# TuringLang/AdvancedVI.jl

Hardware: AMD Instinct MI355X
Metric: ELBO-grad-estimates/sec (higher is better)
Workload: dtype f32

## Files before the change

### advancedvi.jl_amd/csrc/kernels_fullrank_batch.hip

```cpp
#include <algorithm>
#include <cstdlib>
#include <type_traits>
#include <cstdio>
#include <vector>

#include "device_common.h"
#include "fr_elem.h"
#include "fr_planes.h"

#ifndef FB_VK
#define FB_VK 0
#endif
#ifndef FB_WJ
#define FB_WJ 1
#endif

namespace mivi {

struct FbArgs {
  int d, M, L;
  int dT, MT;
  const float *params;
  const float *t_mean, *t_istd;
  unsigned *CA;
  float *cscale;
  unsigned *epsP;
  unsigned *WV;
  float *winv;
  const float *t_prec;
  int dP;
  unsigned *PA;
  float *pscale;
  unsigned *RP;
  float *rinv;
  const float *Tinv;
  unsigned *TA;
  float *tscale;
  long long plane_stride;
  double *ell_part;
  long long ell_stride;
  double *he_part;
  long long he_stride;
  double *ld_part;
  const int4 *work;
  int n_work;
  float *grads;
  long long grad_stride;
  float *values;
  long long value_stride;
  float *grad_last, *value_last;
  int lane_last;
  int write_upper;
  int ent_kind, M_total;
  int *status;
  double ell_const;
  RngArgs rng;
  int n_riders;
  int obj;
  float *parts;
  long long part_stride;
  int knock;
  long long *dbg;
};
#ifdef MIVI_DEV
#define FB_STAMP(a, slot) do { if ((a).dbg && threadIdx.x == 0) (a).dbg[(size_t)blockIdx.x * 8 + (slot)] = (long long)wall_clock64(); } while (0)
#define FB_NOTE(a, slot, v) do { if ((a).dbg && threadIdx.x == 0) (a).dbg[(size_t)blockIdx.x * 8 + (slot)] = (long long)(v); } while (0)
#define FB_KNOCKED(a, b) ((a).knock & (b))
#else
#define FB_KNOCKED(a, b) false
#define FB_STAMP(a, slot) do { } while (0)
#define FB_NOTE(a, slot, v) do { } while (0)
#endif

template <int NT, class Ld4, class Ld>
__device__ __forceinline__ void fb_rowblock_planes(int d, int rb, int kg_lo, int kg_hi, int sub, int nsub, Ld4 ld4, Ld ld, unsigned *planes, float *scale, float *red) {
  constexpr int NP = NT / 8, NW = NT / 64;
  const int tid = threadIdx.x, r4 = tid & 7, part = tid >> 3, ng = d >> 4;
  f32x4 m = {0.f, 0.f, 0.f, 0.f};
  {
    int k = 16 * kg_lo + part;
    for (; k + 7 * NP <= 16 * kg_hi + 15; k += 8 * NP) {
      f32x4 v[8];
#pragma unroll
      for (int u = 0; u < 8; ++u) v[u] = ld4(k + NP * u, 32 * rb + 4 * r4);
#pragma unroll
      for (int u = 0; u < 8; ++u)
#pragma unroll
        for (int c = 0; c < 4; ++c) m[c] = fmaxf(m[c], fabsf(v[u][c]));
    }
    for (; k <= 16 * kg_hi + 15; k += NP) {
      const f32x4 v = ld4(k, 32 * rb + 4 * r4);
#pragma unroll
      for (int c = 0; c < 4; ++c) m[c] = fmaxf(m[c], fabsf(v[c]));
    }
  }
#pragma unroll
  for (int c = 0; c < 4; ++c) {
    m[c] = fmaxf(m[c], __shfl_xor(m[c], 8, 64));
    m[c] = fmaxf(m[c], __shfl_xor(m[c], 16, 64));
    m[c] = fmaxf(m[c], __shfl_xor(m[c], 32, 64));
  }
  if ((tid & 63) < 8) *(f32x4 *)(red + (tid >> 6) * 32 + 4 * r4) = m;
  lds_barrier();
  const int w = tid >> 6, lane = tid & 63, l31 = lane & 31, h = lane >> 5;
  float mm = red[l31];
#pragma unroll
  for (int p = 1; p < NW; ++p) mm = fmaxf(mm, red[p * 32 + l31]);
  float s, inv;
  fb_scale_of(mm, s, inv);
  if (sub == 0 && tid < 32) {
    scale[32 * rb + tid] = s;
    scale[d + 32 * rb + tid] = inv;
  }
  for (int kg = kg_lo + w + NW * sub; kg <= kg_hi; kg += NW * nsub) {
    float x[8];
#pragma unroll
    for (int e = 0; e < 8; ++e) x[e] = ld(16 * kg + 8 * (e >> 2) + 4 * h + (e & 3), 32 * rb + l31) * s;
    fb_store_frag(planes + ((size_t)rb * ng + kg) * kFrag + 4 * lane, x);
  }
}
template <int NT>
__device__ __forceinline__ void fb_cplanes_block(const FbArgs &a, int rb, int sub, int nsub, float *red) {
  const int d = a.d, ng = d >> 4, dT = a.dT;
  const float *C = a.params + dT;
  const int hi = 2 * rb + 3 < ng - 1 ? 2 * rb + 3 : ng - 1;
  if (dT == d) {
    fb_rowblock_planes<NT>(d, rb, 0, hi, sub, nsub,
                       [C, d](int k, int row) { f32x4 v = *(const f32x4 *)(C + (size_t)k * d + row);
#pragma unroll
                                                for (int c = 0; c < 4; ++c) v[c] = k > row + c ? 0.f : v[c];
                                                return v; },
                       [C, d](int k, int row) { const float v = C[(size_t)k * d + row]; return k > row ? 0.f : v; }, a.CA, a.cscale, red);
    return;
  }
  fb_rowblock_planes<NT>(d, rb, 0, hi, sub, nsub,
                     [C, dT](int k, int row) { const bool in = row < dT && k < dT;
                                               f32x4 v = *(const f32x4 *)(C + (size_t)(in ? k : 0) * dT + (in ? row : 0));
#pragma unroll
                                               for (int c = 0; c < 4; ++c) v[c] = (!in || k > row + c) ? 0.f : v[c];
                                               return v; },
                     [C, dT](int k, int row) { if (row >= dT || k > row) return 0.f; return C[(size_t)k * dT + row]; }, a.CA, a.cscale, red);
}
__global__ __launch_bounds__(512) void k_fb_pplanes(FbArgs a) {
  __shared__ float red[8 * 32];
  const float *P = a.t_prec;
  const int dP = a.dP;
  fb_rowblock_planes<512>(a.d, (int)blockIdx.x, 0, (a.d >> 4) - 1, (int)blockIdx.y, (int)gridDim.y,
                     [P, dP](int k, int row) { return *(const f32x4 *)(P + (size_t)k * dP + row); },
                     [P, dP](int k, int row) { return P[(size_t)k * dP + row]; }, a.PA, a.pscale, red);
}
__global__ __launch_bounds__(512) void k_fb_tplanes(FbArgs a) {
  __shared__ float red[8 * 32];
  const float *T = a.Tinv;
  const int d = a.d, rb = (int)blockIdx.x;
  fb_rowblock_planes<512>(d, rb, 2 * (rb & ~3), (d >> 4) - 1, (int)blockIdx.y, (int)gridDim.y,
                     [T, d](int k, int row) { f32x4 v = *(const f32x4 *)(T + (size_t)k * d + row);
#pragma unroll
                                              for (int c = 0; c < 4; ++c) v[c] = k >= row + c ? v[c] : 0.f;
                                              return v; },
                     [T, d](int k, int row) { const float v = T[(size_t)k * d + row]; return k >= row ? v : 0.f; }, a.TA, a.tscale, red);
}

__global__ __launch_bounds__(512) void k_fb_eps(FbArgs a) {
  __shared__ double red[128];
  const int tid = threadIdx.x, d = a.d;
  if ((int)blockIdx.y < a.n_riders) {
    const int r = (int)blockIdx.y * (int)gridDim.x + (int)blockIdx.x;
    if (r < 4 * (d >> 5)) fb_cplanes_block<512>(a, (d >> 5) - 1 - (r >> 2), r & 3, 4, (float *)red);
    return;
  }
  const int l = (int)blockIdx.y - a.n_riders, eb = 2 * (int)blockIdx.x + (tid >> 8);
  const uint64_t idx = rng_index(a.rng) + (a.obj ? 0ull : (uint64_t)l);
  const int moff = a.rng.m_offset + (a.obj ? l * a.MT : 0);
  unsigned *epsP = a.epsP + (size_t)l * a.plane_stride;
  const int nrb6 = d >> 6;
  const int R64 = eb % nrb6, c32 = eb / nrb6;
  const int lane = tid & 63, l31 = lane & 31, h = lane >> 5, f = (tid >> 6) & 3;
  const int rm = c32 * 32 + l31;
  const uint64_t q0 = (uint64_t)(moff + rm) * (uint64_t)(a.dT >> 2);
  float x[8], he = 0.f;
#pragma unroll
  for (int b = 0; b < 2; ++b) {
    const int ri = R64 * 64 + 4 * (4 * f + 2 * b + h);
    float e[4];
    eps_block<float>(a.rng.seed, idx, q0 + (uint64_t)(ri >> 2), e);
    if (!(ri < a.dT && rm < a.MT)) { e[0] = 0.f; e[1] = 0.f; e[2] = 0.f; e[3] = 0.f; }
#pragma unroll
    for (int r = 0; r < 4; ++r) x[4 * b + r] = e[r] * kEpsScale;
    he += 0.5f * (e[0] * e[0] + e[1] * e[1] + e[2] * e[2] + e[3] * e[3]);
  }
  fb_store_frag(epsP + ((size_t)c32 * (d >> 4) + 4 * R64 + f) * kFrag + 4 * lane, x);
  const float hw = wave_sum_f32(he);
  if (lane == 0) red[tid >> 6] = (double)hw;
  lds_barrier();
  if ((tid & 255) == 0) {
    const double *r4 = red + 4 * (tid >> 8);
    a.he_part[(size_t)l * a.he_stride + eb] = ((r4[0] + r4[1]) + r4[2]) + r4[3];
  }
}

constexpr int kImgW = 32 * 36;
template <int WJ>
__device__ __forceinline__ void fb_sched_interleave() {
  constexpr int NM = 6 * WJ, ND = 4 + 2 * WJ, NV = 2 * WJ;
  static_for<0, NM>([&](auto K) {
    constexpr int k = decltype(K)::value;
    constexpr int nrd = (k + 1) * ND / NM - k * ND / NM;
    __builtin_amdgcn_sched_group_barrier(0x008, 1, 0);
    if constexpr (nrd > 0) __builtin_amdgcn_sched_group_barrier(0x100, nrd, 0);
    if constexpr (k < NV) __builtin_amdgcn_sched_group_barrier(0x020, 1, 0);
  });
}
using FbI0 = std::integral_constant<int, 0>;
using FbI1 = std::integral_constant<int, 1>;
using FbI2 = std::integral_constant<int, 2>;
using FbI3 = std::integral_constant<int, 3>;
using FbT = std::true_type;
using FbN = std::false_type;

template <int MASK>
__device__ __forceinline__ float fb_lane_max(float v) {
#pragma unroll
  for (int o = 1; o < 64; o <<= 1)
    if (MASK & o) v = fmaxf(v, __shfl_xor(v, o, 64));
  return v;
}

enum { FB_DIAG = 0, FB_DENSE_R = 1, FB_DENSE_G = 2, FB_STL_U = 3 };
template <int WJ, int MODE, int NRP>
__global__ __launch_bounds__(512 / WJ, (MODE == 2 && NRP == 4 && WJ == 1) ? 4 : 2 / WJ) void k_fb_prod(FbArgs a) {
  constexpr bool kDG = MODE == FB_DENSE_G, kSU = MODE == FB_STL_U, kDR = MODE == FB_DENSE_R;
  constexpr int LDC = 36, NF = WJ, kPW = 2 * WJ;
  constexpr int NW = 8 / WJ, NWN = 4 / WJ;
  constexpr int kBody = (NRP * kStageW > 16 * kImgW) ? NRP * kStageW : 16 * kImgW;
  constexpr bool kTabInBody = kDG && NRP * kStageW + 2048 <= kBody;
  constexpr int kTab = kDG ? (kTabInBody ? 128 : 2048 + 128) : 0;
  __shared__ __attribute__((aligned(16))) unsigned lds[kBody + 4 * 128 + NW * 64 + kTab];
  float *vec = reinterpret_cast<float *>(lds + kBody);
  float *red = vec + 4 * 128;
  float *rsv = red + NW * 64;
  float *tab = kTabInBody ? reinterpret_cast<float *>(lds + NRP * kStageW) : rsv + 128;
  const int tid = threadIdx.x, lane = tid & 63, l31 = lane & 31, h = lane >> 5;
  const int w = __builtin_amdgcn_readfirstlane(tid >> 6);
  const int wm = w / NWN, wn = w % NWN;
  const __attribute__((address_space(4))) int *wp = (const __attribute__((address_space(4))) int *)a.work + 4 * blockIdx.x;
  const int ln = wp[0], rc = wp[1], flags = wp[2];
  const int rb = rc & 0xffff, cb = rc >> 16;
  const int d = a.d, ng = d >> 4;
  const int row0 = rb * 128, col0 = cb * 128;
  const int R0 = row0 >> 5;
  const int g0 = kSU ? 2 * R0 : 0;
  const int G = kDG ? ng : (kSU ? ng - g0 : 2 * (R0 + 4));
  const unsigned *sp[NF];
  int gmax[NF];
#pragma unroll
  for (int f = 0; f < NF; ++f) {
    const int fs = NF * w + f, fr = fs & 3;
    if (fs < 4) {
      sp[f] = (kDG ? a.PA : (kSU ? a.TA : a.CA)) + ((size_t)(R0 + fr) * ng + g0) * kFrag + 4 * lane;
      gmax[f] = (!kDG && !kSU && 2 * (R0 + fr) + 3 < G - 1) ? 2 * (R0 + fr) + 3 : G - 1;
    } else {
      sp[f] = (kDG ? a.RP : a.epsP) + (size_t)ln * a.plane_stride + ((size_t)((col0 >> 5) + fr) * ng + g0) * kFrag + 4 * lane;
      gmax[f] = G - 1;
    }
  }
  int gd = 0;
  constexpr int kMaxNB = 16;
  float tv[4] = {0.f, 0.f, 0.f, 0.f}, tri[kDG ? kMaxNB : 1], trs = 0.f;
  auto load_tables = [&]() {
    if (tid < 128) {
      if constexpr (!kDG && !kSU) {
        const bool in = row0 + tid < a.dT;
        tv[0] = in ? a.params[row0 + tid] : 0.f;
        tv[1] = in ? a.t_mean[row0 + tid] : 0.f;
        if (MODE == FB_DIAG) tv[2] = in ? a.t_istd[row0 + tid] : 0.f;
      }
      const float *sc = kDG ? a.pscale : (kSU ? a.tscale : a.cscale);
      tv[3] = sc[d + row0 + tid];
      if constexpr (kDG) {
        const float *ri = a.rinv + (size_t)ln * (size_t)(d >> 7) * a.M + col0 + tid;
        const int NB = d >> 7;
#pragma unroll
        for (int b = 0; b < kMaxNB; ++b) tri[b] = ri[(size_t)(b < NB ? b : NB - 1) * a.M];
        trs = ri[(size_t)rb * a.M];
      }
    }
    asm volatile("" ::: "memory");
  };
  auto stage_tables = [&]() {
    if (tid < 128) {
      if constexpr (!kDG && !kSU) {
        vec[tid] = tv[0];
        vec[128 + tid] = tv[1];
        if (MODE == FB_DIAG) vec[256 + tid] = tv[2];
      }
      vec[384 + tid] = tv[3] * ((kDG) ? 1.f : kEpsInv);
      if constexpr (kDG) {
        const int NB = d >> 7;
        float u = tri[0], grow = 1.f;
#pragma unroll
        for (int b = 1; b < kMaxNB; ++b) {
          if (b < NB) {
            float ratio = u / tri[b];
            if (!(ratio <= 1099511627776.f)) ratio = 1099511627776.f;
            if (ratio > 1.f && grow * ratio > 1.2089258e24f) ratio = fmaxf(1.2089258e24f / grow, 1.f);
            if (ratio > 1.f) grow *= ratio;
            tab[(b - 1) * 128 + tid] = ratio;
            u = u / ratio;
          }
        }
        tab[(NB - 1) * 128 + tid] = u;
        rsv[tid] = trs;
      }
    }
  };
  auto issue = [&](int slot) {
#pragma unroll
    for (int f = 0; f < NF; ++f) {
      unsigned *dst = lds + slot * kStageW + (NF * w + f) * 512;
      FB_GLDS16(sp[f], dst, 0);
      FB_GLDS16(sp[f], dst, 1024);
      sp[f] += gd < gmax[f] ? kFrag : 0;
    }
    ++gd;
  };
  f32x16 acc[2][WJ];
#pragma unroll
  for (int i = 0; i < 2; ++i)
#pragma unroll
    for (int j = 0; j < WJ; ++j)
#pragma unroll
      for (int r = 0; r < 16; ++r) acc[i][j][r] = 0.f;
  const int r32[2] = {R0 + 2 * wm, R0 + 2 * wm + 1};
  const int Gw = (kDG || kSU) ? G : 2 * r32[1] + 2;
  auto after_group = [&](auto S, int g) {
    if constexpr (kDG && (decltype(S)::value & 3) == 3) {
      if (((g + 1) & 7) == 0) {
#pragma unroll
        for (int j = 0; j < WJ; ++j) {
          const float f = tab[((g >> 3) << 7) + 32 * (WJ * wn + j) + l31];
#pragma unroll
          for (int i = 0; i < 2; ++i) {
#pragma unroll
            for (int r = 0; r < 16; ++r) acc[i][j][r] *= f;
          }
        }
        asm volatile("" ::: "memory");
      }
    }
  };
  auto compute = [&](auto S, int g, const FbFrags<WJ> &F) {
    if (!FB_KNOCKED(a, 2)) fb_group<WJ>(F, acc);
    fb_sched_interleave<WJ>();
    after_group(S, g);
  };
  const unsigned lds0 = (unsigned)(uintptr_t)lds + 16u * lane;
  const unsigned ab_lo = lds0 + (2 * wm) * 2 * 1024, bb_lo = lds0 + (8 + WJ * wn * 2) * 1024;
  const unsigned ab_hi = ab_lo + 4 * kStageW * 4, bb_hi = bb_lo + 4 * kStageW * 4;
  (void)ab_hi; (void)bb_hi;
  auto step = [&](auto S, auto VM, auto ISS, int g, const FbFrags<WJ> &Fc, FbFrags<WJ> &Fn) {
    constexpr int sl = decltype(S)::value;
    fb_wait_vm<kPW * decltype(VM)::value>();
    if (!FB_KNOCKED(a, 8)) fb_barrier();
#ifdef MIVI_SB
    __builtin_amdgcn_sched_barrier(0);
#endif
    auto group_and_read = [&]() {
#ifndef MIVI_DEV
      if constexpr (WJ == 1) {
        constexpr int nx = (sl + 1) % NRP, off = (nx & 3) * kStageW * 4;
        fb_group_read_asm<off>(acc[0][0], acc[1][0], Fc, Fn, nx < 4 ? ab_lo : ab_hi, nx < 4 ? bb_lo : bb_hi);
        if constexpr (kDG && (sl & 3) == 3) {
          if (((g + 1) & 7) == 0) asm volatile("s_nop 15\n\ts_nop 7" : "+v"(acc[0][0]), "+v"(acc[1][0])::"memory");
        }
        after_group(S, g);
      } else
#endif
      {
        if (!FB_KNOCKED(a, 4)) fb_read_frags<WJ>(lds, (sl + 1) % NRP, wm, wn, lane, Fn);
        compute(S, g, Fc);
      }
    };
    if constexpr (decltype(ISS)::value) {
      if (!FB_KNOCKED(a, 1)) issue(sl);
      group_and_read();
    } else if (g < Gw) {
      group_and_read();
    }
  };
  FB_STAMP(a, 0);
  FB_NOTE(a, 4, G);
  load_tables();
  static_for<0, NRP>([&](auto S) { issue(decltype(S)::value); });
  fb_wait_vm<kPW * NRP>();
  stage_tables();
  fb_wait_vm<kPW * (NRP - 1)>();
  fb_barrier();
  FB_STAMP(a, 1);
  {
    FbFrags<WJ> F0, F1;
    fb_read_frags<WJ>(lds, 0, wm, wn, lane, F0);
    int g = 0;
    for (; g + NRP < G; g += NRP) {
      static_for<0, NRP>([&](auto S) {
        constexpr int sv = decltype(S)::value;
        if constexpr (sv % 2 == 0) step(S, std::integral_constant<int, NRP - 2>{}, FbT{}, g + sv, F0, F1);
        else step(S, std::integral_constant<int, NRP - 2>{}, FbT{}, g + sv, F1, F0);
      });
    }
    static_for<0, NRP - 1>([&](auto S) {
      constexpr int sv = decltype(S)::value;
      if constexpr (sv % 2 == 0) step(S, std::integral_constant<int, NRP - 2 - sv>{}, FbN{}, g + sv, F0, F1);
      else step(S, std::integral_constant<int, NRP - 2 - sv>{}, FbN{}, g + sv, F1, F0);
    });
    __builtin_amdgcn_s_waitcnt(0xc07f);
    if (g + NRP - 1 < Gw) compute(std::integral_constant<int, NRP - 1>{}, g + NRP - 1, F1);
  }
  f32x16 (&tot)[2][WJ] = acc;
  fb_barrier();
  FB_STAMP(a, 2);
  float *img = reinterpret_cast<float *>(lds) + w * (2 * WJ * kImgW);
  unsigned *WVl = a.WV + (size_t)ln * a.plane_stride;
  unsigned *RPl = a.RP + (size_t)ln * a.plane_stride;
  double *ellp = a.ell_part + (size_t)ln * a.ell_stride;
  const int ncb = a.M >> 5, nmg = a.M >> 4;
  const int ei4 = 4 * (lane & 7);
  float amax[2][4];
  float cmax[WJ][4];
#pragma unroll
  for (int i = 0; i < 2; ++i)
#pragma unroll
    for (int c = 0; c < 4; ++c) amax[i][c] = 0.f;
#pragma unroll
  for (int j = 0; j < WJ; ++j)
#pragma unroll
    for (int p = 0; p < 4; ++p) cmax[j][p] = 0.f;
#pragma unroll
  for (int i = 0; i < 2; ++i) {
    const int lr = 64 * wm + 32 * i;
    f32x4 mu = {0.f, 0.f, 0.f, 0.f}, tm = mu, tis = mu;
    const f32x4 zf = *(const f32x4 *)(vec + 384 + lr + ei4);
    if constexpr (!kDG && !kSU) {
      mu = *(const f32x4 *)(vec + lr + ei4);
      tm = *(const f32x4 *)(vec + 128 + lr + ei4);
      if constexpr (MODE == FB_DIAG) tis = *(const f32x4 *)(vec + 256 + lr + ei4);
    }
#pragma unroll
    for (int j = 0; j < WJ; ++j) {
      float *I = img + (i * WJ + j) * kImgW;
      const int cb32 = (col0 >> 5) + WJ * wn + j;
      const bool pad = 32 * r32[i] >= a.dT || 32 * cb32 >= a.MT;
#pragma unroll
      for (int q = 0; q < 4; ++q) {
        const f32x4 v = {tot[i][j][4 * q], tot[i][j][4 * q + 1], tot[i][j][4 * q + 2], tot[i][j][4 * q + 3]};
        *(f32x4 *)(I + l31 * LDC + 8 * q + 4 * h) = v;
      }
      if constexpr (kSU) {
        const float uf = vec[384 + lr + l31];
        const float wo = a.winv[(size_t)ln * (size_t)(a.M >> 7) * d + (size_t)cb * d + row0 + lr + l31];
#pragma unroll
        for (int g2 = 0; g2 < 2; ++g2) {
          const unsigned *src = WVl + ((size_t)r32[i] * nmg + 2 * cb32 + g2) * kFrag + 4 * lane;
          const u32x4v wh = *(const u32x4v *)src, wl = *(const u32x4v *)(src + 256);
#pragma unroll
          for (int e = 0; e < 8; ++e) {
            float *p = I + (16 * g2 + 8 * (e >> 2) + 4 * h + (e & 3)) * LDC + l31;
            const float x = __builtin_fmaf(*p, uf, fb_unsplit2(wh, wl, e) * wo);
            *p = x;
            amax[i][0] = fmaxf(amax[i][0], fabsf(x));
          }
        }
        continue;
      }
      double s = 0.0;
#pragma unroll
      for (int p = 0; p < 4; ++p) {
        const int en = 8 * p + (lane >> 3);
        const f32x4 v = *(const f32x4 *)(I + en * LDC + ei4) * zf;
        float ell = 0.f;
        f32x4 wv;
        if constexpr (MODE == FB_DIAG) {
          const f32x4 z = mu + v;
#pragma unroll
          for (int c = 0; c < 4; ++c) wv[c] = diag_target_elem(z[c], tm[c], tis[c], ell);
        } else if constexpr (kDR) {
          const f32x4 z = mu + v;
          wv = z - tm;
        } else {
          const unsigned *fr = RPl + ((size_t)cb32 * ng + 2 * r32[i] + (ei4 >> 4)) * kFrag + 4 * (en + 32 * ((ei4 >> 2) & 1)) + 2 * ((ei4 >> 3) & 1);
          const uint2 qh = *(const uint2 *)fr, ql = *(const uint2 *)(fr + 256);
          const float rs = rsv[32 * (WJ * wn + j) + en];
          const unsigned uh[2] = {qh.x, qh.y}, ul[2] = {ql.x, ql.y};
#pragma unroll
          for (int c = 0; c < 4; ++c) wv[c] = dense_target_elem(v[c], fb_unsplit2_word(uh[c >> 1], ul[c >> 1], c & 1) * rs, ell);
        }
        if (pad) { wv = f32x4{0.f, 0.f, 0.f, 0.f}; ell = 0.f; }
        *(f32x4 *)(I + en * LDC + ei4) = wv;
        if constexpr (kDR) {
          cmax[j][p] = fmaxf(cmax[j][p], fmaxf(fmaxf(fabsf(wv[0]), fabsf(wv[1])), fmaxf(fabsf(wv[2]), fabsf(wv[3]))));
        } else {
#pragma unroll
          for (int c = 0; c < 4; ++c) amax[i][c] = fmaxf(amax[i][c], fabsf(wv[c]));
          const double sv = (double)wave_sum_f32(ell);
          s = p ? s + sv : sv;
        }
      }
      if constexpr (!kDR) {
        if (lane == 0) ellp[(size_t)r32[i] * ncb + cb32] = s;
      }
    }
  }
  if constexpr (kDR) {
#pragma unroll
    for (int j = 0; j < WJ; ++j)
#pragma unroll
      for (int p = 0; p < 4; ++p) {
        const float m = fb_lane_max<7>(cmax[j][p]);
        if ((lane & 7) == 0) red[w * 64 + 32 * j + 8 * p + (lane >> 3)] = m;
      }
  } else if constexpr (kSU) {
#pragma unroll
    for (int i = 0; i < 2; ++i) {
      const float m = fb_lane_max<32>(amax[i][0]);
      if (lane < 32) red[w * 64 + 32 * i + lane] = m;
    }
  } else {
#pragma unroll
    for (int i = 0; i < 2; ++i)
#pragma unroll
      for (int c = 0; c < 4; ++c) {
        const float m = fb_lane_max<56>(amax[i][c]);
        if (lane < 8) red[w * 64 + 32 * i + ei4 + c] = m;
      }
  }
  fb_barrier();
  if constexpr (kDR) {
#pragma unroll
    for (int j = 0; j < WJ; ++j) {
      const int cb32 = (col0 >> 5) + WJ * wn + j;
      float s, inv;
      fb_scale_of(fmaxf(red[wn * 64 + 32 * j + l31], red[(NWN + wn) * 64 + 32 * j + l31]), s, inv);
      if (wm == 0 && lane < 32) a.rinv[(size_t)ln * (size_t)(d >> 7) * a.M + (size_t)rb * a.M + col0 + 32 * (WJ * wn + j) + lane] = inv;
#pragma unroll
      for (int i = 0; i < 2; ++i) {
        const float *I = img + (i * WJ + j) * kImgW;
#pragma unroll
        for (int g2 = 0; g2 < 2; ++g2) {
          const f32x4 x0 = *(const f32x4 *)(I + l31 * LDC + 16 * g2 + 4 * h) * s, x1 = *(const f32x4 *)(I + l31 * LDC + 16 * g2 + 8 + 4 * h) * s;
          const float x[8] = {x0[0], x0[1], x0[2], x0[3], x1[0], x1[1], x1[2], x1[3]};
          fb_store_frag(RPl + ((size_t)cb32 * ng + 2 * r32[i] + g2) * kFrag + 4 * lane, x);
        }
      }
    }
  } else {
#pragma unroll
    for (int i = 0; i < 2; ++i) {
      float mx = red[(wm * NWN) * 64 + 32 * i + l31];
#pragma unroll
      for (int x = 1; x < NWN; ++x) mx = fmaxf(mx, red[(wm * NWN + x) * 64 + 32 * i + l31]);
      float s, inv;
      fb_scale_of(mx, s, inv);
      if (wn == 0 && lane < 32) a.winv[(size_t)ln * (size_t)(a.M >> 7) * d + (size_t)cb * d + row0 + 64 * wm + 32 * i + lane] = inv;
#pragma unroll
      for (int j = 0; j < WJ; ++j) {
        const float *I = img + (i * WJ + j) * kImgW;
        const int cb32 = (col0 >> 5) + WJ * wn + j;
#pragma unroll
        for (int g2 = 0; g2 < 2; ++g2) {
          float x[8];
#pragma unroll
          for (int e = 0; e < 8; ++e) x[e] = I[(16 * g2 + 8 * (e >> 2) + 4 * h + (e & 3)) * LDC + l31] * s;
          fb_store_frag(WVl + ((size_t)r32[i] * nmg + 2 * cb32 + g2) * kFrag + 4 * lane, x);
        }
      }
    }
  }
  FB_STAMP(a, 3);
  if (!kDG && !kSU && (flags & 1) && wn == 0 && lane < 32) {
    const int nrb = d >> 5;
#pragma unroll
    for (int i = 0; i < 2; ++i) {
      const int r = 32 * r32[i] + lane;
      float lg, bad;
      logdet_block32(r < a.dT ? a.params[a.dT + (size_t)r * a.dT + r] : 1.f, lg, bad);
      if (lane == 0) {
        a.ld_part[r32[i]] = (double)lg;
        a.ld_part[nrb + r32[i]] = (double)bad;
      }
    }
  }
}

__device__ __forceinline__ void fb_value_block(const FbArgs &a, int l, double *red) {
  const int d = a.d;
  ValueIn vin{};
  vin.ell_const = a.ell_const;
  vin.ell_part = a.ell_part + (size_t)l * a.ell_stride;
  vin.n_ell_part = (d >> 5) * (a.M >> 5);
  vin.he_part = a.he_part + (size_t)l * a.he_stride;
  vin.n_he_part = (d >> 6) * (a.M >> 5);
  vin.ld_part = a.ld_part;
  vin.n_ld_part = d >> 5;
  OutArgs out{};
  const bool last = l == a.lane_last && a.value_last;
  out.value = last ? a.value_last : a.values + (size_t)l * a.value_stride;
  if (a.parts) {
    out.partials_mode = 1;
    out.partials = a.parts + (size_t)l * a.part_stride;
    out.scalars_off = (int64_t)d + (int64_t)(d >> 7) * ((d >> 7) + 1) / 2 * 16384;
  }
  out.ent_kind = a.ent_kind;
  out.M_total = a.M_total;
  out.M_local = a.MT;
  out.status = a.status;
  const float *pp = a.params;
  const int dT = a.dT;
  finalize_value_block<float, 256, false>(dT, vin, out, (int64_t)dT + (int64_t)dT * dT, [pp, dT](int i) { return pp[dT + (size_t)i * dT + i]; }, red);
}

template <int WJ, int NRV, int TABW, int WPE, bool PART = false>
__global__ __launch_bounds__(512 / WJ, WPE / WJ) void k_fb_vjp(FbArgs a) {
  static_assert(WJ == 1, "the transposing B reads are written for the 64 x 32 wave tiles");
  constexpr int LDC = 36, NF = WJ, kPW = 2 * WJ;
  constexpr int NR = NRV;
  constexpr int kBody = (NR * kStageW > 16 * kImgW / 2) ? NR * kStageW : 16 * kImgW / 2;
  __shared__ __attribute__((aligned(16))) unsigned lds[kBody + TABW];
  float *wf = reinterpret_cast<float *>(lds + kBody);
  const int tid = threadIdx.x, lane = tid & 63, l31 = lane & 31, h = lane >> 5;
  const int w = __builtin_amdgcn_readfirstlane(tid >> 6);
  const int wm = w / (4 / WJ), wn = w % (4 / WJ);
  if ((int)blockIdx.x < a.L) {
    if (tid < 256) fb_value_block(a, (int)blockIdx.x, reinterpret_cast<double *>(lds));
    return;
  }
  const __attribute__((address_space(4))) int *wp = (const __attribute__((address_space(4))) int *)a.work + 4 * ((int)blockIdx.x - a.L);
  const int ln = wp[0], rc = wp[1];
  const int rb = rc & 0xffff, cb = rc >> 16;
  const int d = a.d, M = a.M, nmg = M >> 4, dT = a.dT;
  const int row0 = rb * 128, col0 = cb * 128;
  const bool last = ln == a.lane_last && a.grad_last;
  float *grad = last ? a.grad_last : a.grads + (size_t)ln * a.grad_stride;
  const bool upper = a.write_upper || last;
  const int G = nmg;
  const int NB = M >> 7;
  const unsigned *sp[NF];
  unsigned btr;
  {
    const int G4 = lane >> 4, c16 = lane & 15;
    const int kgpar = G4 & 1, hq = G4 >> 1, hp = c16 & 1, half = (c16 >> 1) & 1, sl = 4 * hq + (c16 >> 2);
    btr = 16u * (unsigned)(8 * (2 * hp + kgpar) + ((sl & 7) ^ (4 * hp))) + 8u * (unsigned)half;
  }
#pragma unroll
  for (int f = 0; f < NF; ++f) {
    const int fs = NF * w + f, fr = fs & 3;
    if (fs < 4) {
      sp[f] = a.WV + (size_t)ln * a.plane_stride + ((size_t)((row0 >> 5) + fr) * nmg) * kFrag + 4 * lane;
    } else {
      const int m8 = lane >> 3, s8 = m8 >> 2, hp = (m8 >> 1) & 1, kgpar = m8 & 1, sl = 8 * s8 + ((lane & 7) ^ (4 * hp));
      sp[f] = a.epsP + (size_t)ln * a.plane_stride + ((size_t)((col0 >> 4) + 2 * fr + kgpar)) * kFrag + 4 * (sl + 32 * hp);
    }
  }
  int gi = 0;
  const int bstep_odd = (d >> 4) * kFrag - 64;
  constexpr int kMaxNBv = 16;
  float twi[kMaxNBv];
  auto load_table = [&]() {
    if (tid < 128) {
      const float *wi = a.winv + (size_t)ln * (size_t)NB * d + row0 + tid;
#pragma unroll
      for (int r = 0; r < kMaxNBv; ++r) twi[r] = wi[(size_t)(r < NB ? r : NB - 1) * d];
    }
    asm volatile("" ::: "memory");
  };
  auto build_table = [&]() {
    if (tid < 128) {
      float u = twi[0], grow = 1.f;
#pragma unroll
      for (int r = 1; r < kMaxNBv; ++r) {
        if (r < NB) {
          float ratio = u / twi[r];
          if (!(ratio <= 1099511627776.f)) ratio = 1099511627776.f;
          if (ratio > 1.f && grow * ratio > 1.2089258e24f) ratio = fmaxf(1.2089258e24f / grow, 1.f);
          if (ratio > 1.f) grow *= ratio;
          wf[(r - 1) * 128 + tid] = ratio;
          u = u / ratio;
        }
      }
      wf[(NB - 1) * 128 + tid] = u;
    }
  };
  auto issue = [&](int slot) {
#pragma unroll
    for (int f = 0; f < NF; ++f) {
      unsigned *dst = lds + slot * kStageW + (NF * w + f) * 512;
      if (!(FB_VK & 16)) {
        FB_GLDS16(sp[f], dst, 0);
        FB_GLDS16(sp[f], dst, 1024);
      }
      if (NF * w + f >= 4) sp[f] += (gi & 1) ? bstep_odd : 64;
      else sp[f] += kFrag;
    }
    ++gi;
  };
  auto read_frags = [&](int slot, FbFrags<WJ> &F) {
    if ((FB_VK & 64)) return;
    const unsigned *cur = lds + slot * kStageW + 4 * lane;
#pragma unroll
    for (int i = 0; i < 2; ++i)
#pragma unroll
      for (int p = 0; p < 2; ++p) F.A[i][p] = *(const u32x4v *)(cur + ((2 * wm + i) * 2 + p) * 256);
    const unsigned bb = (unsigned)(uintptr_t)(lds + slot * kStageW) + (8 + 2 * wn) * 1024 + btr;
    uint2 t0, t1, t2, t3;
    asm volatile("ds_read_b64_tr_b16 %0, %4\n\tds_read_b64_tr_b16 %1, %4 offset:512\n\tds_read_b64_tr_b16 %2, %4 offset:1024\n\t"
                 "ds_read_b64_tr_b16 %3, %4 offset:1536\n\ts_waitcnt lgkmcnt(0)"
                 : "=&v"(t0), "=&v"(t1), "=&v"(t2), "=&v"(t3) : "v"(bb) : "memory");
    F.B[0][0] = u32x4v{t0.x, t0.y, t1.x, t1.y};
    F.B[0][1] = u32x4v{t2.x, t2.y, t3.x, t3.y};
  };
  const int ri[2] = {(row0 >> 5) + 2 * wm, (row0 >> 5) + 2 * wm + 1};
  int cj[WJ];
#pragma unroll
  for (int j = 0; j < WJ; ++j) cj[j] = (col0 >> 5) + WJ * wn + j;
  const bool work = cj[0] <= ri[1];
  bool dg[2];
#pragma unroll
  for (int i = 0; i < 2; ++i) {
    dg[i] = false;
#pragma unroll
    for (int j = 0; j < WJ; ++j) dg[i] = dg[i] || ri[i] == cj[j];
  }
  f32x16 acc[2][WJ];
#pragma unroll
  for (int i = 0; i < 2; ++i)
#pragma unroll
    for (int j = 0; j < WJ; ++j)
#pragma unroll
      for (int r = 0; r < 16; ++r) acc[i][j][r] = 0.f;
  double rsd[2] = {0.0, 0.0};
  float rcur[2] = {0.f, 0.f};
  auto after_group = [&](auto S, int g, const FbFrags<WJ> &F) {
    if (__builtin_expect(dg[0] || dg[1], 0)) {
#pragma unroll
      for (int i = 0; i < 2; ++i)
        if (dg[i]) {
#pragma unroll
          for (int e = 0; e < 8; ++e) rcur[i] += fb_unsplit2(F.A[i][0], F.A[i][1], e);
        }
    }
    if constexpr (decltype(S)::value == 3 || decltype(S)::value == -1) {
      if (((g + 1) & 7) == 0 && g + 1 < G) {
        const float *wr = wf + ((g >> 3) << 7) + 64 * wm;
#pragma unroll
        for (int i = 0; i < 2; ++i) {
#pragma unroll
          for (int q = 0; q < 4; ++q) {
            const f32x4 f4 = *(const f32x4 *)(wr + 32 * i + 8 * q + 4 * h);
#pragma unroll
            for (int j = 0; j < WJ; ++j)
#pragma unroll
              for (int c = 0; c < 4; ++c) acc[i][j][4 * q + c] *= f4[c];
          }
          rsd[i] = (rsd[i] + (double)rcur[i]) * (double)wr[32 * i + l31];
          rcur[i] = 0.f;
        }
        asm volatile("" ::: "memory");
      }
    }
  };
  auto compute = [&](auto S, int g, const FbFrags<WJ> &F) {
    if (!(FB_VK & 32)) fb_group<WJ>(F, acc);
    after_group(S, g, F);
  };
  {
    FB_STAMP(a, 0);
    FB_NOTE(a, 4, G);
    load_table();
#pragma unroll
    for (int s0 = 0; s0 < NR - 1; ++s0) issue(s0);
    fb_wait_vm<kPW * (NR - 1)>();
    build_table();
    int slot = 0;
    for (int g = 0; g < G; ++g) {
      if (g == 1) FB_STAMP(a, 1);
      if (g + NR - 2 < G) fb_wait_vm<kPW * (NR - 2)>();
      else if (NR > 3 && g + 1 < G) fb_wait_vm<kPW>();
      else fb_wait_vm<0>();
      fb_barrier();
      if (g + NR - 1 < G) issue(slot == 0 ? NR - 1 : slot - 1);
      if (work) {
        FbFrags<WJ> F;
        read_frags(slot, F);
        compute(std::integral_constant<int, -1>{}, g, F);
      }
      slot = slot == NR - 1 ? 0 : slot + 1;
    }
  }
  fb_barrier();
  FB_STAMP(a, 2);
  if ((FB_VK & 128)) return;
  float *Cs = reinterpret_cast<float *>(lds) + w * kImgW;
  const float *wfin = wf + (NB - 1) * 128 + 64 * wm;
  const double invM = 1.0 / (double)a.M_total;
  const bool pow2M = (a.M_total & (a.M_total - 1)) == 0;
  const float invMe = (float)invM * kEpsInv;
  const double direct = direct_entropy_coeff(a.ent_kind);
  const int i4 = 4 * (lane & 7);
#pragma unroll
  for (int i = 0; i < 2; ++i) {
#pragma unroll
    for (int j = 0; j < WJ; ++j) {
      if (cj[j] > ri[i] || 32 * ri[i] >= dT) continue;
      const bool diag = ri[i] == cj[j];
      const int rbase = 32 * ri[i], cbase = 32 * cj[j];
#pragma unroll
      for (int q = 0; q < 4; ++q) {
        const f32x4 v = {acc[i][j][4 * q], acc[i][j][4 * q + 1], acc[i][j][4 * q + 2], acc[i][j][4 * q + 3]};
        *(f32x4 *)(Cs + l31 * LDC + 8 * q + 4 * h) = v;
      }
      const f32x4 ff = *(const f32x4 *)(wfin + 32 * i + i4);
#pragma unroll
      for (int p = 0; p < 4; ++p) {
        const int n = 8 * p + (lane >> 3);
        const int gi = rbase + i4, gj = cbase + n;
        float cjj = 1.f;
        if (diag && gj >= gi && gj < gi + 4) cjj = a.params[dT + (size_t)gj * dT + gj];
        const f32x4 v = *(const f32x4 *)(Cs + n * LDC + i4) * ff;
        f32x4 o;
        if constexpr (PART) {
          o = v * kEpsInv;
          if (diag) {
#pragma unroll
            for (int c = 0; c < 4; ++c) o[c] = gj > gi + c ? 0.f : o[c];
          }
          store16_wt(a.parts + (size_t)ln * a.part_stride + d + ((size_t)(rb * (rb + 1) / 2 + cb) << 14) + (size_t)(gj - col0) * 128 + (gi - row0), o);
          continue;
        }
        if (!diag && pow2M) {
          o = -v * invMe;
        } else {
#pragma unroll
          for (int c = 0; c < 4; ++c) o[c] = vjp_elem(v[c] * kEpsInv, gi + c, gj, pow2M, (float)invM, invM, direct, cjj);
        }
        store16_wt(grad + dT + (size_t)gj * dT + gi, o);
      }
      if (!PART && !diag && upper) {
        const f32x4 z4 = {0.f, 0.f, 0.f, 0.f};
#pragma unroll
        for (int p = 0; p < 4; ++p) {
          const int ii = 8 * p + (lane >> 3);
          store16_wt(grad + dT + (size_t)(rbase + ii) * dT + cbase + i4, z4);
        }
      }
      asm volatile("s_waitcnt lgkmcnt(0)" ::: "memory");
    }
    if (dg[i] && 32 * ri[i] < dT) {
      const double mine = (rsd[i] + (double)rcur[i]) * (double)wfin[32 * i + l31];
      const double sm = mine + __shfl_xor(mine, 32, 64);
      if constexpr (PART) {
        if (lane < 32) a.parts[(size_t)ln * a.part_stride + 32 * ri[i] + lane] = (float)sm;
      } else {
        if (lane < 32) grad[32 * ri[i] + lane] = dmu_elem(sm, invM);
      }
    }
  }
  FB_STAMP(a, 3);
}

__global__ __launch_bounds__(256) void k_fb_finalize_parts(FbArgs a) {
  __shared__ double red[4 * 4];
  const int d = a.d, l = blockIdx.y, j = blockIdx.x, tid = threadIdx.x;
  const float *P = a.parts + (size_t)l * a.part_stride;
  const bool last = l == a.lane_last && a.grad_last;
  float *grad = last ? a.grad_last : a.grads + (size_t)l * a.grad_stride;
  const bool upper = a.write_upper || last;
  const double invM = 1.0 / (double)a.M_total;
  const bool pow2M = (a.M_total & (a.M_total - 1)) == 0;
  const double direct = direct_entropy_coeff(a.ent_kind);
  if (j == d) {
    for (int i = tid; i < d; i += 256) grad[i] = dmu_elem((double)P[i], invM);
    double s_ld = 0.0, bad = 0.0;
    for (int i = tid; i < d; i += 256) {
      const double c = (double)a.params[d + (size_t)i * d + i];
      if (!(c > 0.0)) bad = 1.0;
      s_ld += log(c);
    }
    double v[2] = {s_ld, bad};
    block_sum_n<double, 256, 2>(v, red);
    if (tid == 0) {
      const int64_t so = (int64_t)d + (int64_t)(d >> 7) * ((d >> 7) + 1) / 2 * 16384;
      const double sum_ell = (double)P[so], s_he = (double)P[so + 1], Mt = (double)a.M_total;
      const double ent = (ent_is_closed(a.ent_kind) ? 0.5 * d * (1.0 + kLog2Pi) : s_he / Mt + 0.5 * d * kLog2Pi) + v[0];
      const double value = -(sum_ell / Mt + ent);
      float *vo = (l == a.lane_last && a.value_last) ? a.value_last : a.values + (size_t)l * a.value_stride;
      *vo = (float)value;
      int st = 0;
      if (!isfinite(value)) st |= 1;
      if (v[1] > 0.0) st |= 2;
      if (st && a.status) atomicOr(a.status, st);
    }
    return;
  }
  const int cb = j >> 7, lj = j & 127;
  const float cjj = a.params[d + (size_t)j * d + j];
  for (int i4 = 4 * tid; i4 < d; i4 += 1024) {
    f32x4 o = {0.f, 0.f, 0.f, 0.f};
    if (i4 + 3 >= j) {
      const int rb = i4 >> 7;
      const f32x4 v = *(const f32x4 *)(P + d + ((size_t)(rb * (rb + 1) / 2 + cb) << 14) + (size_t)lj * 128 + (i4 & 127));
#pragma unroll
      for (int c = 0; c < 4; ++c) o[c] = vjp_elem(v[c], i4 + c, j, pow2M, (float)invM, invM, direct, cjj);
    } else if (!upper) {
      continue;
    }
    *(f32x4 *)(grad + d + (size_t)j * d + i4) = o;
  }
}

namespace {
constexpr int kBM = 128, kBN = 128;
constexpr int kWJ = FB_WJ;
constexpr int kOwnCuTilesPerCU10 = 17;
}

static int fb_pad(int x) { return (x + 127) / 128 * 128; }
bool fb_shape_ok(const mivi_ctx *c, int M) {
  static const bool off = getenv("MIVI_BATCH_GEN3") && atoi(getenv("MIVI_BATCH_GEN3")) == 0;
  return !off && c->cfg.family == MIVI_FULLRANK && c->cfg.dtype == MIVI_F32 && c->cfg.d % 32 == 0 && M % 32 == 0 && c->cfg.d >= kBM &&
         c->cfg.d <= 2048 && M >= 128 && M <= 2048;
}
bool fb_whole_tiles(const mivi_ctx *c, int M) { return c->cfg.d % kBM == 0 && M % kBN == 0; }
size_t fb_plane_words(const mivi_ctx *c, int M) { return (size_t)fb_pad(c->cfg.d) * fb_pad(M) / 512 * kFrag; }
size_t fb_cplane_words(const mivi_ctx *c) { return (size_t)(fb_pad(c->cfg.d) / 32) * (fb_pad(c->cfg.d) / 16) * kFrag; }
size_t fb_part_len(const mivi_ctx *c) {
  const size_t d = (size_t)c->cfg.d, T = d / 128;
  return (d + T * (T + 1) / 2 * 16384 + 2 + 3) / 4 * 4;
}

const FbTab *fb_prepare(mivi_ctx *c, int M, int L) {
  FbTables &ft = c->fb;
  for (FbTab &t : ft.tab)
    if (t.L == L && t.M == M && t.prod.p && t.vjp.p) return &t;
  FbTab &t = ft.tab[ft.next_tab];
  ft.next_tab = (ft.next_tab + 1) & 3;
  invalidate_graph(c);
  (void)hipStreamSynchronize(c->stream);
  t.L = t.M = 0;
  const int d = fb_pad(c->cfg.d), nrb = d / kBM, ncb = fb_pad(M) / kBN;
  std::vector<std::vector<int4>> lists(8);
  int panel = 0;
  for (int l = 0; l < L; ++l)
    for (int cb = 0; cb < ncb; ++cb, ++panel)
      for (int rb = nrb - 1; rb >= 0; --rb) lists[panel % 8].push_back(make_int4(l, rb | (cb << 16), (l == 0 && cb == 0) ? 1 : 0, 0));
  while (true) {
    int a = 0, b = 0;
    for (int x = 1; x < 8; ++x) {
      if (lists[x].size() > lists[a].size()) a = x;
      if (lists[x].size() < lists[b].size()) b = x;
    }
    if (lists[a].size() <= lists[b].size() + 1) break;
    lists[b].push_back(lists[a].back());
    lists[a].pop_back();
  }
  for (auto &li : lists) std::stable_sort(li.begin(), li.end(), [](const int4 &p, const int4 &q) { return (p.y & 0xffff) > (q.y & 0xffff); });
  std::vector<int4> prod;
  size_t mx = 0;
  for (auto &li : lists) mx = std::max(mx, li.size());
  for (size_t i = 0; i < mx; ++i)
    for (int x = 0; x < 8; ++x)
      if (i < lists[x].size()) prod.push_back(lists[x][i]);
  std::vector<int4> flat;
  for (int l = 0; l < L; ++l)
    for (int rb = 0; rb < nrb; ++rb)
      for (int cb = 0; cb <= rb; ++cb) flat.push_back(make_int4(l, rb | (cb << 16), 0, 0));
  std::vector<int4> vjp;
  {
    const size_t n = flat.size();
    size_t pos = 0;
    std::vector<std::vector<int4>> lx(8);
    for (int x = 0; x < 8; ++x) {
      const size_t e = (n * (x + 1)) / 8;
      for (; pos < e; ++pos) lx[x].push_back(flat[pos]);
    }
    size_t m2 = 0;
    for (auto &li : lx) m2 = std::max(m2, li.size());
    for (size_t i = 0; i < m2; ++i)
      for (int x = 0; x < 8; ++x)
        if (i < lx[x].size()) vjp.push_back(lx[x][i]);
  }
  std::vector<int4> prod2;
  const size_t panel_bytes = (size_t)kBM * d * 4;
  constexpr int NG = 4, NC = 8 / NG;
  if (nrb % NG == 0 && (size_t)(nrb / NG) * panel_bytes <= (1u << 20)) {
    std::vector<std::vector<int4>> lp(8);
    int pn = 0;
    for (int l = 0; l < L; ++l)
      for (int cb = 0; cb < ncb; ++cb, ++pn)
        for (int rg = 0; rg < NG; ++rg)
          for (int r = 0; r < nrb / NG; ++r) lp[rg + NG * (pn % NC)].push_back(make_int4(l, (rg * (nrb / NG) + r) | (cb << 16), 0, 0));
    size_t m3 = 0;
    for (auto &li : lp) m3 = std::max(m3, li.size());
    for (size_t i = 0; i < m3; ++i)
      for (int x = 0; x < 8; ++x)
        if (i < lp[x].size()) prod2.push_back(lp[x][i]);
  } else {
    for (int l = 0; l < L; ++l)
      for (int cb = 0; cb < ncb; ++cb)
        for (int rb = 0; rb < nrb; ++rb) prod2.push_back(make_int4(l, rb | (cb << 16), 0, 0));
  }
  std::vector<int4> prod3;
  for (auto &li : lists) std::stable_sort(li.begin(), li.end(), [](const int4 &p, const int4 &q) { return (p.y & 0xffff) < (q.y & 0xffff); });
  for (size_t i = 0; i < mx; ++i)
    for (int x = 0; x < 8; ++x)
      if (i < lists[x].size()) prod3.push_back(lists[x][i]);
  if (upload(c, t.prod, prod.data(), prod.size() * sizeof(int4)) || upload(c, t.vjp, vjp.data(), vjp.size() * sizeof(int4)) ||
      upload(c, t.prod2, prod2.data(), prod2.size() * sizeof(int4)) || upload(c, t.prod3, prod3.data(), prod3.size() * sizeof(int4)))
    return nullptr;
  t.n_prod2 = (int)prod2.size();
  t.n_prod = (int)prod.size();
  t.n_vjp = (int)vjp.size();
  t.L = L;
  t.M = M;
  return &t;
}

static FbArgs fb_args(mivi_ctx *c, const void *params, int M_true) {
  FbTables &t = c->fb;
  const int d = fb_pad(c->cfg.d), M = fb_pad(M_true);
  FbArgs a{};
  a.d = d; a.M = M;
  a.dT = c->cfg.d; a.MT = M_true;
  a.params = (const float *)params;
  a.t_mean = (const float *)c->t_mean.p;
  a.t_istd = (const float *)c->t_istd.p;
  a.CA = (unsigned *)t.CA.p;
  a.cscale = (float *)t.cscale.p;
  a.pscale = (float *)t.pscale.p;
  a.tscale = (float *)t.tscale.p;
  a.winv = (float *)t.winv.p;
  a.rinv = (float *)t.rinv.p;
  a.epsP = (unsigned *)t.epsP.p;
  a.WV = (unsigned *)t.WV.p;
  a.t_prec = (const float *)c->t_prec.p; a.dP = c->dP;
  a.PA = (unsigned *)t.PA.p;
  a.RP = (unsigned *)t.RP.p;
  a.Tinv = (const float *)t.Tinv.p;
  a.TA = (unsigned *)t.TA.p;
  a.plane_stride = (long long)fb_plane_words(c, M);
  a.ell_part = (double *)t.ell.p; a.ell_stride = (long long)(d / 32) * (M / 32);
  a.he_part = (double *)t.he.p; a.he_stride = (long long)(d / 64) * (M / 32);
  a.ld_part = (double *)t.ld.p;
  a.ent_kind = c->cfg.entropy; a.M_total = c->M_total;
  a.status = (int *)c->status.p;
  a.ell_const = c->t_const;
  return a;
}

void fb_launch_eps(mivi_ctx *c, const FbStep &s, bool with_cplanes, hipStream_t stream) {
  const int d = fb_pad(c->cfg.d), M = fb_pad(s.M), L = s.L;
  FbArgs a = fb_args(c, s.params, s.M);
  a.L = L;
  a.rng = s.rng;
  a.obj = s.obj;
  const int gx = (d / 64) * (M / 32) / 2;
  a.n_riders = with_cplanes ? (4 * (d / 32) + gx - 1) / gx : 0;
  hipLaunchKernelGGL(k_fb_eps, dim3(gx, L + a.n_riders), dim3(512), 0, stream, a);
}
void fb_launch_pplanes(mivi_ctx *c, hipStream_t stream) {
  FbArgs a = fb_args(c, nullptr, c->cfg.n_mc);
  hipLaunchKernelGGL(k_fb_pplanes, dim3(c->cfg.d / 32, 4), dim3(512), 0, stream, a);
}
void fb_launch_tplanes(mivi_ctx *c, hipStream_t stream) {
  FbArgs a = fb_args(c, nullptr, c->cfg.n_mc);
  hipLaunchKernelGGL(k_fb_tplanes, dim3(c->cfg.d / 32, 4), dim3(512), 0, stream, a);
}
void fb_launch_compute(mivi_ctx *c, const FbStep &s, hipStream_t stream, int which) {
  const FbTab &tb = *s.tab;
  FbArgs a = fb_args(c, s.params, s.M);
  a.L = s.L;
  a.grads = (float *)s.grads; a.grad_stride = s.grad_stride;
  a.values = (float *)s.values; a.value_stride = s.value_stride;
  a.grad_last = (float *)s.grad_last; a.value_last = (float *)s.value_last; a.lane_last = s.lane_last;
  a.write_upper = s.write_upper;
  a.parts = (float *)s.parts; a.part_stride = s.part_stride;
  if (s.obj) { a.ent_kind = s.ent_kind; a.M_total = s.M; }
#ifdef MIVI_DEV
  static long long *dbg_buf = nullptr;
  static const bool dbg_on = getenv("MIVI_FB_DBG") != nullptr;
  if (dbg_on && !dbg_buf) (void)hipMalloc(&dbg_buf, 2 * 8192 * 8 * sizeof(long long));
  auto dump = [&](const char *name, int n) {
    if (!dbg_on) return;
    (void)hipStreamSynchronize(stream);
    std::vector<long long> h((size_t)n * 8);
    (void)hipMemcpy(h.data(), dbg_buf, h.size() * 8, hipMemcpyDeviceToHost);
    long long t0 = h[0], t3 = 0;
    for (int i = 0; i < n; ++i) { t0 = std::min(t0, h[(size_t)i * 8]); t3 = std::max(t3, h[(size_t)i * 8 + 3]); }
    double pro = 0, loop = 0, epi = 0, pg = 0; long long gs = 0;
    for (int i = 0; i < n; ++i) { const long long *r = &h[(size_t)i * 8]; pro += r[1] - r[0]; loop += r[2] - r[1]; epi += r[3] - r[2]; gs += r[4]; }
    pg = loop / (double)gs;
    fprintf(stderr, "[fbdbg] %s: %d workgroups, span %.2f us | mean prologue %.2f us, main loop %.2f us (%.3f us per group), epilogue %.2f us | last start %.2f us\n", name, n, (t3 - t0) * 0.01, pro / n * 0.01, loop / n * 0.01, pg * 0.01, epi / n * 0.01, 0.0);
    std::vector<long long> st; for (int i = 0; i < n; ++i) st.push_back(h[(size_t)i * 8] - t0);
    std::sort(st.begin(), st.end());
    fprintf(stderr, "[fbdbg]   starts (us): p25 %.2f p50 %.2f p75 %.2f p90 %.2f max %.2f\n", st[n / 4] * 0.01, st[n / 2] * 0.01, st[3 * n / 4] * 0.01, st[9 * n / 10] * 0.01, st[n - 1] * 0.01);
  };
  a.dbg = dbg_on ? dbg_buf : nullptr;
  a.knock = getenv("MIVI_FB_KNOCK") ? atoi(getenv("MIVI_FB_KNOCK")) : 0;
#endif
  a.work = (const int4 *)tb.prod.p; a.n_work = tb.n_prod;
  const int n_cu = c->n_cu > 0 ? c->n_cu : 256;
  auto own_cu_for = [&](int n, bool equal_tiles) {
#ifdef MIVI_DEV
    static const int force_ring = getenv("MIVI_FB_RING") ? atoi(getenv("MIVI_FB_RING")) : 0;
    if (force_ring == 4) return false;
    if (force_ring == 8) return true;
#endif
    const int gmax = fb_pad(c->cfg.d) / 16;
    const int thr10 = gmax <= 32 ? 10 : (gmax <= 64 ? 10 + (gmax - 32) * 7 / 32 : kOwnCuTilesPerCU10 + (gmax - 64 < 64 ? gmax - 64 : 64) * 5 / 64);
    return !equal_tiles && n > n_cu && 10 * (long long)n <= (long long)thr10 * n_cu;
  };
  auto prod = [&](auto MODE, int n) {
    constexpr int md = decltype(MODE)::value;
    if (own_cu_for(n, md == FB_DENSE_G)) hipLaunchKernelGGL((k_fb_prod<kWJ, md, 8>), dim3(n), dim3(512 / kWJ), 0, stream, a);
    else hipLaunchKernelGGL((k_fb_prod<kWJ, md, 4>), dim3(n), dim3(512 / kWJ), 0, stream, a);
  };
  if (s.dense) {
    if (which & 1) prod(std::integral_constant<int, FB_DENSE_R>{}, tb.n_prod);
    a.work = (const int4 *)tb.prod2.p; a.n_work = tb.n_prod2;
    if (which & 4) prod(std::integral_constant<int, FB_DENSE_G>{}, tb.n_prod2);
  } else if (which & 1) {
    prod(std::integral_constant<int, FB_DIAG>{}, tb.n_prod);
#ifdef MIVI_DEV
    dump("k_fb_prod<DIAG>", tb.n_prod);
#endif
  }
  if (s.stl && (which & 8)) {
    a.work = (const int4 *)tb.prod3.p; a.n_work = tb.n_prod;
    prod(std::integral_constant<int, FB_STL_U>{}, tb.n_prod);
  }
  a.work = (const int4 *)tb.vjp.p; a.n_work = tb.n_vjp;
  if (s.values_only) {
    if (which & 2) hipLaunchKernelGGL((k_fb_vjp<kWJ, 3, 256, 6>), dim3(s.L), dim3(512 / kWJ), 0, stream, a);
    return;
  }
  if (which & 2) {
    if (s.parts) {
      if (a.M <= 256) hipLaunchKernelGGL((k_fb_vjp<kWJ, 3, 256, 6, true>), dim3(tb.n_vjp + s.L), dim3(512 / kWJ), 0, stream, a);
      else hipLaunchKernelGGL((k_fb_vjp<kWJ, 3, 2048, 4, true>), dim3(tb.n_vjp + s.L), dim3(512 / kWJ), 0, stream, a);
    }
    else if (a.M <= 256) hipLaunchKernelGGL((k_fb_vjp<kWJ, 3, 256, 6>), dim3(tb.n_vjp + s.L), dim3(512 / kWJ), 0, stream, a);
    else hipLaunchKernelGGL((k_fb_vjp<kWJ, 3, 2048, 4>), dim3(tb.n_vjp + s.L), dim3(512 / kWJ), 0, stream, a);
#ifdef MIVI_DEV
    dump("k_fb_vjp", tb.n_vjp);
#endif
  }
}

void fb_launch_finalize_parts(mivi_ctx *c, const FbStep &s, hipStream_t stream) {
  FbArgs a = fb_args(c, s.params, s.M);
  a.L = s.L;
  a.grads = (float *)s.grads; a.grad_stride = s.grad_stride;
  a.values = (float *)s.values; a.value_stride = s.value_stride;
  a.grad_last = (float *)s.grad_last; a.value_last = (float *)s.value_last; a.lane_last = s.lane_last;
  a.write_upper = s.write_upper;
  a.parts = (float *)s.parts; a.part_stride = s.part_stride;
  hipLaunchKernelGGL(k_fb_finalize_parts, dim3(c->cfg.d + 1, s.L), dim3(256), 0, stream, a);
}

}
```

Measured before the change: 358,500.

## Prefetch first fragment during max scan and split loads into uniform/varying offsets

```diff
diff --git a/advancedvi.jl_amd/csrc/kernels_fullrank_batch.hip b/advancedvi.jl_amd/csrc/kernels_fullrank_batch.hip
--- a/advancedvi.jl_amd/csrc/kernels_fullrank_batch.hip
+++ b/advancedvi.jl_amd/csrc/kernels_fullrank_batch.hip
@@ -72,26 +72,53 @@
 #define FB_NOTE(a, slot, v) do { } while (0)
 #endif
 
-template <int NT, class Ld4, class Ld>
-__device__ __forceinline__ void fb_rowblock_planes(int d, int rb, int kg_lo, int kg_hi, int sub, int nsub, Ld4 ld4, Ld ld, unsigned *planes, float *scale, float *red) {
-  constexpr int NP = NT / 8, NW = NT / 64;
-  const int tid = threadIdx.x, r4 = tid & 7, part = tid >> 3, ng = d >> 4;
+template <class T>
+__device__ __forceinline__ T fb_ld_at(const float *base, int iu, int iv) {
+  return *(const T *)((const char *)base + (unsigned)__builtin_amdgcn_readfirstlane(4 * iu) + (unsigned)(4 * iv));
+}
+template <int NT, class Ld4, class M4, class Ld, class M1>
+__device__ __forceinline__ void fb_rowblock_planes(int d, int rb, int kg_lo, int kg_hi, int sub, int nsub, Ld4 ld4, M4 m4, Ld ld, M1 m1, unsigned *planes, float *scale,
+                                                   float *red) {
+  constexpr int NP = NT / 8, NW = NT / 64, NL = 8;
+  const int tid = threadIdx.x, r4 = tid & 7, ng = d >> 4;
+  const int w = __builtin_amdgcn_readfirstlane(tid >> 6), lane = tid & 63, l31 = lane & 31, h = lane >> 5, p8 = lane >> 3;
+  const int k_end = 16 * kg_hi + 15, kg0 = kg_lo + w + NW * sub, kgs = NW * nsub;
+  auto max_ku = [&](int kb, int u) { const int ku = kb + NP * u + 8 * w; return ku <= k_end ? ku : k_end - 7; };
+  auto max_load = [&](f32x4 (&v)[NL], int kb) {
+#pragma unroll
+    for (int u = 0; u < NL; ++u) v[u] = ld4(max_ku(kb, u), p8, 32 * rb + 4 * r4);
+  };
+  auto max_fold = [&](const f32x4 (&v)[NL], int kb, f32x4 &m) {
+#pragma unroll
+    for (int u = 0; u < NL; ++u) {
+      const f32x4 x = m4(v[u], max_ku(kb, u) + p8, 32 * rb + 4 * r4);
+#pragma unroll
+      for (int c = 0; c < 4; ++c) m[c] = fmaxf(m[c], fabsf(x[c]));
+    }
+  };
+  auto frag_load = [&](float (&x)[8], int kg) {
+#pragma unroll
+    for (int e = 0; e < 8; ++e) x[e] = ld(16 * min(kg, kg_hi) + 8 * (e >> 2) + (e & 3), 4 * h, 32 * rb + l31);
+  };
+  auto frag_lay = [&](const float (&x)[8], int kg, float s) {
+    float y[8];
+#pragma unroll
+    for (int e = 0; e < 8; ++e) y[e] = m1(x[e], 16 * kg + 8 * (e >> 2) + 4 * h + (e & 3), 32 * rb + l31) * s;
+    fb_store_frag(planes + ((size_t)rb * ng + kg) * kFrag + 4 * lane, y);
+  };
   f32x4 m = {0.f, 0.f, 0.f, 0.f};
+  float x[8];
   {
-    int k = 16 * kg_lo + part;
-    for (; k + 7 * NP <= 16 * kg_hi + 15; k += 8 * NP) {
-      f32x4 v[8];
-#pragma unroll
-      for (int u = 0; u < 8; ++u) v[u] = ld4(k + NP * u, 32 * rb + 4 * r4);
-#pragma unroll
-      for (int u = 0; u < 8; ++u)
-#pragma unroll
-        for (int c = 0; c < 4; ++c) m[c] = fmaxf(m[c], fabsf(v[u][c]));
-    }
-    for (; k <= 16 * kg_hi + 15; k += NP) {
-      const f32x4 v = ld4(k, 32 * rb + 4 * r4);
-#pragma unroll
-      for (int c = 0; c < 4; ++c) m[c] = fmaxf(m[c], fabsf(v[c]));
+    f32x4 v[NL];
+    int kb = 16 * kg_lo;
+    max_load(v, kb);
+    frag_load(x, kg0);
+    __builtin_amdgcn_sched_barrier(0);
+    max_fold(v, kb, m);
+    for (kb += NL * NP; kb <= k_end; kb += NL * NP) {
+      max_load(v, kb);
+      __builtin_amdgcn_sched_barrier(0);
+      max_fold(v, kb, m);
     }
   }
 #pragma unroll
@@ -102,21 +129,19 @@
   }
   if ((tid & 63) < 8) *(f32x4 *)(red + (tid >> 6) * 32 + 4 * r4) = m;
   lds_barrier();
-  const int w = tid >> 6, lane = tid & 63, l31 = lane & 31, h = lane >> 5;
   float mm = red[l31];
 #pragma unroll
   for (int p = 1; p < NW; ++p) mm = fmaxf(mm, red[p * 32 + l31]);
   float s, inv;
   fb_scale_of(mm, s, inv);
+  if (kg0 <= kg_hi) frag_lay(x, kg0, s);
+  for (int kg = kg0 + kgs; kg <= kg_hi; kg += kgs) {
+    frag_load(x, kg);
+    frag_lay(x, kg, s);
+  }
   if (sub == 0 && tid < 32) {
     scale[32 * rb + tid] = s;
     scale[d + 32 * rb + tid] = inv;
-  }
-  for (int kg = kg_lo + w + NW * sub; kg <= kg_hi; kg += NW * nsub) {
-    float x[8];
-#pragma unroll
-    for (int e = 0; e < 8; ++e) x[e] = ld(16 * kg + 8 * (e >> 2) + 4 * h + (e & 3), 32 * rb + l31) * s;
-    fb_store_frag(planes + ((size_t)rb * ng + kg) * kFrag + 4 * lane, x);
   }
 }
 template <int NT>
@@ -126,42 +151,47 @@
   const int hi = 2 * rb + 3 < ng - 1 ? 2 * rb + 3 : ng - 1;
   if (dT == d) {
     fb_rowblock_planes<NT>(d, rb, 0, hi, sub, nsub,
-                       [C, d](int k, int row) { f32x4 v = *(const f32x4 *)(C + (size_t)k * d + row);
-#pragma unroll
-                                                for (int c = 0; c < 4; ++c) v[c] = k > row + c ? 0.f : v[c];
-                                                return v; },
-                       [C, d](int k, int row) { const float v = C[(size_t)k * d + row]; return k > row ? 0.f : v; }, a.CA, a.cscale, red);
+                       [C, d](int ku, int kv, int row) { return fb_ld_at<f32x4>(C, ku * d, kv * d + row); },
+                       [](f32x4 v, int k, int row) {
+#pragma unroll
+                         for (int c = 0; c < 4; ++c) v[c] = k > row + c ? 0.f : v[c];
+                         return v; },
+                       [C, d](int ku, int kv, int row) { return fb_ld_at<float>(C, ku * d, kv * d + row); },
+                       [](float v, int k, int row) { return k > row ? 0.f : v; }, a.CA, a.cscale, red);
     return;
   }
   fb_rowblock_planes<NT>(d, rb, 0, hi, sub, nsub,
-                     [C, dT](int k, int row) { const bool in = row < dT && k < dT;
-                                               f32x4 v = *(const f32x4 *)(C + (size_t)(in ? k : 0) * dT + (in ? row : 0));
-#pragma unroll
-                                               for (int c = 0; c < 4; ++c) v[c] = (!in || k > row + c) ? 0.f : v[c];
-                                               return v; },
-                     [C, dT](int k, int row) { if (row >= dT || k > row) return 0.f; return C[(size_t)k * dT + row]; }, a.CA, a.cscale, red);
+                     [C, dT](int ku, int kv, int row) { return fb_ld_at<f32x4>(C, (ku < dT ? ku : 0) * dT, kv * dT + min(row, dT - 4)); },
+                     [dT](f32x4 v, int k, int row) { const bool in = row < dT && k < dT;
+#pragma unroll
+                                                     for (int c = 0; c < 4; ++c) v[c] = (!in || k > row + c) ? 0.f : v[c];
+                                                     return v; },
+                     [C, dT](int ku, int kv, int row) { return fb_ld_at<float>(C, (ku < dT ? ku : 0) * dT, kv * dT + min(row, dT - 1)); },
+                     [dT](float v, int k, int row) { return (row >= dT || k > row) ? 0.f : v; }, a.CA, a.cscale, red);
 }
 __global__ __launch_bounds__(512) void k_fb_pplanes(FbArgs a) {
   __shared__ float red[8 * 32];
   const float *P = a.t_prec;
   const int dP = a.dP;
   fb_rowblock_planes<512>(a.d, (int)blockIdx.x, 0, (a.d >> 4) - 1, (int)blockIdx.y, (int)gridDim.y,
-                     [P, dP](int k, int row) { return *(const f32x4 *)(P + (size_t)k * dP + row); },
-                     [P, dP](int k, int row) { return P[(size_t)k * dP + row]; }, a.PA, a.pscale, red);
+                     [P, dP](int ku, int kv, int row) { return fb_ld_at<f32x4>(P, ku * dP, kv * dP + row); }, [](f32x4 v, int, int) { return v; },
+                     [P, dP](int ku, int kv, int row) { return fb_ld_at<float>(P, ku * dP, kv * dP + row); }, [](float v, int, int) { return v; }, a.PA, a.pscale, red);
 }
 __global__ __launch_bounds__(512) void k_fb_tplanes(FbArgs a) {
   __shared__ float red[8 * 32];
   const float *T = a.Tinv;
   const int d = a.d, rb = (int)blockIdx.x;
   fb_rowblock_planes<512>(d, rb, 2 * (rb & ~3), (d >> 4) - 1, (int)blockIdx.y, (int)gridDim.y,
-                     [T, d](int k, int row) { f32x4 v = *(const f32x4 *)(T + (size_t)k * d + row);
-#pragma unroll
-                                              for (int c = 0; c < 4; ++c) v[c] = k >= row + c ? v[c] : 0.f;
-                                              return v; },
-                     [T, d](int k, int row) { const float v = T[(size_t)k * d + row]; return k >= row ? v : 0.f; }, a.TA, a.tscale, red);
-}
-
-__global__ __launch_bounds__(512) void k_fb_eps(FbArgs a) {
+                     [T, d](int ku, int kv, int row) { return fb_ld_at<f32x4>(T, ku * d, kv * d + row); },
+                     [](f32x4 v, int k, int row) {
+#pragma unroll
+                       for (int c = 0; c < 4; ++c) v[c] = k >= row + c ? v[c] : 0.f;
+                       return v; },
+                     [T, d](int ku, int kv, int row) { return fb_ld_at<float>(T, ku * d, kv * d + row); },
+                     [](float v, int k, int row) { return k >= row ? v : 0.f; }, a.TA, a.tscale, red);
+}
+
+__global__ __launch_bounds__(512) __attribute__((amdgpu_waves_per_eu(8))) void k_fb_eps(FbArgs a) {
   __shared__ double red[128];
   const int tid = threadIdx.x, d = a.d;
   if ((int)blockIdx.y < a.n_riders) {
```

New measurement: 361,100, median of 6. Within noise of the previous version (+0.7%).
